# UniBwTAS/continuous_clustering

Hardware: AMD Instinct MI355X
Metric: Mpoints/s clustered (64-beam streams) (higher is better)
Workload: dtype f32

## Files before the change

### continuous_clustering_amd/__init__.py

```python
from __future__ import annotations

import ctypes as C
import os
import sys

import numpy as np

from . import capi
from .capi import Config

__all__ = ["Config", "Engine", "EngineError", "load_library", "capi", "IDENTITY_TF", "take", "TAKE_POINT_DTYPE", "TAKE_STREAM_DTYPE",
           "TakeCapacityError", "pointcloud2_fields", "TAKE_CLUSTER_DTYPE", "TAKE_CLUSTER_STREAM_DTYPE", "poses", "PoseTracks",
           "stamps", "FiringStamps", "CLUSTER_STAMP_DTYPE"]

_HERE = os.path.dirname(os.path.abspath(__file__))
LIB_PATH = os.path.join(_HERE, os.environ.get("CC_HIP_LIB", "libcc_hip.so"))
_lib = None

IDENTITY_TF = np.array([1, 0, 0, 0, 0, 1, 0, 0, 0, 0, 1, 0], dtype=np.float64)


class EngineError(RuntimeError):
    def __init__(self, code: int, msg: str):
        super().__init__(f"cc_hip error {code}: {msg}")
# ... 10 lines not shown
            return
        libdir = os.path.join(list(spec.submodule_search_locations)[0], "lib")
        for name in ("libhsa-runtime64.so", "libamdhip64.so"):
            path = os.path.join(libdir, name)
            if os.path.exists(path):
                C.CDLL(path, mode=C.RTLD_GLOBAL)
    except OSError:
        pass


def load_library():
    global _lib
    if _lib is not None:
        return _lib
    if not os.path.exists(LIB_PATH):
        raise ImportError(f"{LIB_PATH} is missing: build it with `python -m continuous_clustering_amd.build` "
                          f"(hipcc --offload-arch=gfx950); there is no CPU fallback")
    _preload_hip_runtime()
    L = C.CDLL(LIB_PATH)
    vp, i32, i64 = C.c_void_p, C.c_int, C.c_int64
    L.cc_config_default.argtypes = [C.POINTER(Config)]
    L.cc_config_default.restype = None
    L.cc_config_kitti.argtypes = [C.POINTER(Config)]
    L.cc_config_kitti.restype = None
    L.cc_version.restype = C.c_char_p
    L.cc_engine_create.argtypes = [C.POINTER(vp), i32, i32, i32, C.POINTER(Config)]
    L.cc_engine_destroy.argtypes = [vp]
    L.cc_engine_destroy.restype = None
    L.cc_engine_set_config.argtypes = [vp, C.POINTER(Config)]
    L.cc_engine_reset.argtypes = [vp, i32]
    L.cc_engine_reset_streams.argtypes = [vp, i32, vp]
    L.cc_engine_set_robot_from_sensor.argtypes = [vp, i32, vp]
    L.cc_engine_add_firings.argtypes = [vp, i32, i64, vp, vp, vp]
    L.cc_engine_add_firings_device.argtypes = [vp, i64, vp, vp, vp]
    L.cc_engine_sync.argtypes = [vp]
    L.cc_engine_inputs_released.argtypes = [vp, C.POINTER(C.c_uint64), C.POINTER(C.c_uint64)]
    L.cc_engine_hip_stream.argtypes = [vp]
    L.cc_engine_hip_stream.restype = vp
    L.cc_engine_record_events.argtypes = [vp, i32]
    L.cc_engine_drain_events.argtypes = [vp, i32, vp, i64, C.POINTER(i64)]
    L.cc_engine_pending_events.argtypes = [vp, i32, C.POINTER(i64)]
    L.cc_engine_drain_links.argtypes = [vp, i32, vp, i64, C.POINTER(i64)]
    L.cc_engine_stream_state.argtypes = [vp, i32, C.POINTER(capi.StreamState)]
    L.cc_engine_read_columns.argtypes = [vp, i32, i64, i64, C.POINTER(capi.ColumnView)]
    L.cc_engine_read_column_ranges.argtypes = [vp, i32, i32, vp, vp, C.POINTER(capi.ColumnView)]
    L.cc_engine_output_planes.argtypes = [vp, i32, C.POINTER(vp), C.POINTER(vp)]
    L.cc_engine_set_option.argtypes = [vp, C.c_char_p, i64]
    L.cc_engine_gather_cluster_points.argtypes = [vp, i32, i64, vp, vp, vp, vp, vp, vp]
    L.cc_engine_enable_timing.argtypes = [vp, i32]
    L.cc_engine_kernel_times.argtypes = [vp, C.POINTER(C.c_double * 7), C.POINTER(C.c_uint64)]
    L.cc_engine_totals.argtypes = [vp] + [C.POINTER(C.c_uint64)] * 4
    L.cc_engine_batch_counters.argtypes = [vp] + [C.POINTER(C.c_uint64)] * 2 + [C.POINTER(C.c_uint64 * 8)]
    L.cc_engine_gate_counters.argtypes = [vp] + [C.POINTER(C.c_uint64)] * 2
    L.cc_engine_resident_counters.argtypes = [vp, C.POINTER(C.c_uint64), C.POINTER(C.c_uint64), C.POINTER(C.c_int)]
    L.cc_engine_view_counters.argtypes = [vp, C.POINTER(C.c_uint64), C.POINTER(C.c_uint64)]
    L.cc_engine_last_error.argtypes = [vp]
    L.cc_engine_last_error.restype = C.c_char_p
    _lib = L
    return L


def _ptr(a):
    if a is None:
        return None
    if isinstance(a, int):
        return a
    if isinstance(a, np.ndarray):
        return a.ctypes.data
    return a.data_ptr()


class Engine:

    def __init__(self, cfg: Config, num_rows: int, num_streams: int = 1, device: int = 0, robot_from_sensor=IDENTITY_TF):
        self.L = load_library()
        self.cfg = cfg.copy()
        self.num_rows = num_rows
        self.num_streams = num_streams
        self.h = C.c_void_p()
        rc = self.L.cc_engine_create(C.byref(self.h), device, num_streams, num_rows, C.byref(self.cfg))
        if rc != capi.CC_OK:
            self.h = None
            raise EngineError(rc, "cc_engine_create failed" + (" (no MI355X visible)" if rc == capi.CC_ERR_NO_DEVICE else ""))
        if robot_from_sensor is not None:
            self.set_robot_from_sensor(robot_from_sensor)

    def close(self):
        if getattr(self, "h", None):
            self.L.cc_engine_destroy(self.h)
            self.h = None

    def __del__(self):
        try:
            self.close()
        except Exception:
            pass

    def _check(self, rc: int):
        if rc != capi.CC_OK:
            raise EngineError(rc, self.L.cc_engine_last_error(self.h).decode())

    def set_config(self, cfg: Config):
        self.cfg = cfg.copy()
        self._check(self.L.cc_engine_set_config(self.h, C.byref(self.cfg)))

    def reset(self, num_rows: int | None = None):
# ... 80 lines not shown
        a = np.ascontiguousarray(ev["a"], dtype=np.int64)
        b = np.ascontiguousarray(ev["b"], dtype=np.int64)
        cnt = np.ascontiguousarray(ev["d"], dtype=np.uint32)
        offsets = np.zeros(n + 1, dtype=np.int64)
        offsets[1:] = np.cumsum(cnt.astype(np.int64))
        gcol = np.zeros(max(1, int(offsets[-1])), dtype=np.int64)
        row = np.zeros(max(1, int(offsets[-1])), dtype=np.int32)
        self._check(self.L.cc_engine_gather_cluster_points(self.h, stream, n, cid.ctypes.data, a.ctypes.data, b.ctypes.data,
                                                           cnt.ctypes.data, gcol.ctypes.data, row.ctypes.data))
        return offsets, gcol[: offsets[-1]], row[: offsets[-1]]

    def set_option(self, name: str, value: int):
        self._check(self.L.cc_engine_set_option(self.h, name.encode(), int(value)))

    def enable_timing(self, enable: bool = True):
        self._check(self.L.cc_engine_enable_timing(self.h, 1 if enable else 0))

    def kernel_times(self) -> dict:
        ms = (C.c_double * 7)()
        n = C.c_uint64(0)
        self._check(self.L.cc_engine_kernel_times(self.h, C.byref(ms), C.byref(n)))
        names = ("prep_ms", "insert_ms", "segment_ms", "scan_ms", "assoc_lds_ms", "assoc_global_ms", "publish_ms")
        d = {k: ms[i] for i, k in enumerate(names)}
        d["batches"] = n.value
        return d

    def totals(self) -> dict:
        v = [C.c_uint64(0) for _ in range(4)]
        self._check(self.L.cc_engine_totals(self.h, *[C.byref(x) for x in v]))
        return {"cells_published": v[0].value, "clusters_finished": v[1].value, "firings_consumed": v[2].value,
                "serial_columns": v[3].value}

    def batch_counters(self) -> dict:
        v = [C.c_uint64(0) for _ in range(2)]
        why = (C.c_uint64 * 8)()
        self._check(self.L.cc_engine_batch_counters(self.h, *[C.byref(x) for x in v], C.byref(why)))
        return {"batch_columns": v[0].value, "batch_bails": v[1].value, "bail_reasons": list(why)}

    def resident_counters(self) -> dict:
        a, b, r = C.c_uint64(0), C.c_uint64(0), C.c_int(0)
        self._check(self.L.cc_engine_resident_counters(self.h, C.byref(a), C.byref(b), C.byref(r)))
        return {"launches": int(a.value), "calls": int(b.value), "running": bool(r.value)}

    def view_counters(self) -> dict:
        a, b = C.c_uint64(0), C.c_uint64(0)
        self._check(self.L.cc_engine_view_counters(self.h, C.byref(a), C.byref(b)))
        return {"mirror": int(a.value), "kernel": int(b.value)}

    def gate_counters(self) -> dict:
        v = [C.c_uint64(0) for _ in range(2)]
        self._check(self.L.cc_engine_gate_counters(self.h, *[C.byref(x) for x in v]))
        return {"lazy_batches": v[0].value, "lazy_redone": v[1].value}

    def output_planes(self, stream: int = 0):
        g, i = C.c_void_p(), C.c_void_p()
        self._check(self.L.cc_engine_output_planes(self.h, stream, C.byref(g), C.byref(i)))
        return g.value, i.value


from . import take
from .take import TAKE_POINT_DTYPE, TAKE_STREAM_DTYPE, TakeCapacityError, pointcloud2_fields
from .take import TAKE_CLUSTER_DTYPE, TAKE_CLUSTER_STREAM_DTYPE

Engine.take_points = take.take_points
Engine.take_size = take.take_size
Engine.take_cursor = take.take_cursor
Engine.take_seek = take.take_seek
Engine.take_clusters = take.take_clusters
Engine.take_clusters_size = take.take_clusters_size
Engine.take_clusters_cursor = take.take_clusters_cursor

from . import poses
from .poses import PoseTracks

from . import stamps
from .stamps import CLUSTER_STAMP_DTYPE, FiringStamps
```

### continuous_clustering_amd/csrc/cc_engine.hip

```cpp
#include <hip/hip_runtime.h>

#include <algorithm>
#include <chrono>
#include <cstdlib>
#include <cmath>
#include <cstdio>
#include <cstring>
#include <functional>
#include <limits>
#include <mutex>
#include <string>
#include <vector>

#include "cc_kernels.h"

#ifndef CC_LWAVE_MAX_STREAMS
#define CC_LWAVE_MAX_STREAMS 256
#endif

using namespace ccd;

struct cc_engine
{
    int device{0};
// ... 2651 lines not shown
    if (!e || stream < 0 || stream >= e->g.num_streams || slots < 1 || !d_original_index || !d_is_ground || !d_detection || max_points < 1 ||
        from < 0 || to - from >= e->g.ring_cols)
        return CC_ERR_INVALID_ARGUMENT;
    if (to < from)
        return CC_OK;
    (void) hipSetDevice(e->device);
    int rc = stop_resident(e);
    if (rc)
        return rc;
    rc = finish_batch(e);
    if (rc)
        return rc;
    hipLaunchKernelGGL(cck::k_scatter_apply, dim3((unsigned) (to - from + 1)), dim3(64), 0, e->stream, e->g, e->P, (const StreamState*) e->d_states, stream, (long long) from,
                       d_original_index, slots, d_is_ground, d_detection, (long long) max_points);
    CC_HIP_CHECK(e, hipGetLastError());
    return CC_OK;
}

int cc_engine_view_counters(cc_engine* e, uint64_t* served_from_mirror, uint64_t* served_by_kernel)
{
    if (!e)
        return CC_ERR_INVALID_ARGUMENT;
    if (served_from_mirror)
        *served_from_mirror = e->view_hits;
    if (served_by_kernel)
        *served_by_kernel = e->view_misses;
    return CC_OK;
}

int cc_engine_resident_counters(cc_engine* e, uint64_t* launches, uint64_t* calls, int* running)
{
    if (!e)
        return CC_ERR_INVALID_ARGUMENT;
    if (launches)
        *launches = e->res_launches;
    if (calls)
        *calls = e->res_calls + (e->res_running ? __atomic_load_n(&e->h_res_ctl->calls, __ATOMIC_ACQUIRE) : 0ull);
    if (running)
        *running = (e->res_running && __atomic_load_n(&e->h_res_ctl->exited, __ATOMIC_ACQUIRE) == 0ull) ? 1 : 0;
    return CC_OK;
}

int cc_engine_gate_counters(cc_engine* e, uint64_t* lazy_batches, uint64_t* lazy_redone)
{
    if (!e)
        return CC_ERR_INVALID_ARGUMENT;
    if (lazy_batches)
        *lazy_batches = e->lazy_batches;
    if (lazy_redone)
        *lazy_redone = e->lazy_redone;
    return CC_OK;
}

int cc_engine_batch_counters(cc_engine* e, uint64_t* batch_columns, uint64_t* batch_bails, uint64_t bail_reasons[8])
{
    if (!e)
        return CC_ERR_INVALID_ARGUMENT;
    (void) hipSetDevice(e->device);
    int rc = finish_batch(e);
    if (rc)
        return rc;
    std::vector<StreamState> st(e->g.num_streams);
    CC_HIP_CHECK(e, hipMemcpy(st.data(), e->d_states, st.size() * sizeof(StreamState), hipMemcpyDeviceToHost));
    uint64_t a = 0, b = 0;
    if (bail_reasons)
        for (int i = 0; i < 8; i++)
            bail_reasons[i] = 0;
    for (auto& s : st)
    {
        a += s.batch_columns;
        b += s.batch_bails;
        if (bail_reasons)
            for (int i = 0; i < 8; i++)
                bail_reasons[i] += s.batch_bail_reason[i];
    }
    if (bail_reasons)
        bail_reasons[7] = e->small_tail_launches;
    if (batch_columns)
        *batch_columns = a;
    if (batch_bails)
        *batch_bails = b;
    return CC_OK;
}

int cc_engine_debug_counters(cc_engine* e, int stream, uint64_t out[16])
{
    if (!e || stream < 0 || stream >= e->g.num_streams || !out)
        return CC_ERR_INVALID_ARGUMENT;
    StreamState st;
    CC_HIP_CHECK(e, hipMemcpy(&st, e->d_states + stream, sizeof(st), hipMemcpyDeviceToHost));
    for (int i = 0; i < 16; i++)
        out[i] = st.dbg[i];
    return CC_OK;
}

const char* cc_engine_last_error(cc_engine* e)
{
    return e ? e->error.c_str() : "null engine";
}

}

#include "cc_replay_eval.h"
```

### continuous_clustering_amd/csrc/cc_k_scan.h

```cpp
#pragma once

#ifndef CC_SCAN_BLOCKS
#define CC_SCAN_BLOCKS 256
#endif
constexpr int SCAN_BLOCKS = CC_SCAN_BLOCKS;

template<int RPL, bool MIRROR>
__device__ __forceinline__ void scan_body(const Geometry& g, const cc_config& cfg, const Planes& P, StreamState* states, int first_stream, int slot,
                                          const int bx, const int by, const int ny)
{
    const int s = first_stream + bx;
    const int lane = lane_id();
    const StreamState* st = &states[s];
    if (st->error != 0 || st->batch[slot].seg_begin < 0 || st->batch[slot].mode != 0)
        return;
    AssocCtx c;
    c.p = stream_ptrs(P, g, s);
    const SP& p = c.p;
    const int R = c.R = g.num_rows;
    c.NC = g.num_columns;
    const int RC = c.RC = g.ring_cols;
    c.az_width = g.az_width;
    c.maxd2 = g.max_distance_squared;
    c.max_steps_in_row = cfg.max_steps_in_row;
// ... 399 lines not shown
            visits++;
            reach = sb;
        }
        if (ccm::absf(o.w - me.w) > mad)
            next_direction(c);
        else
        {
            const float dx = me.x - o.x, dy = me.y - o.y, dz = me.z - o.z;
            if (!oign && dx * dx + dy * dy + dz * dz < c.maxd2)
            {
                const int cand = (sb << 8) | orow;
                if (!rooted)
                    parent = cand;
                else if (nlinks < LINK_SLOTS)
                {
                    packed |= (unsigned long long) cand << (16 * nlinks);
                    nlinks++;
                }
                else
                    overflow = 1;
                rooted = 1;
            }
            if (rooted && c.stop_enabled && d >= c.stop_min)
                next_direction(c);
            else
            {
                d++;
                orow = down ? orow + 1 : orow - 1;
                if (!(orow >= 0 && orow < c.R && d <= c.max_col_steps))
                    next_direction(c);
            }
        }
    }
};

constexpr int SL_CAP = 8192;
struct ScanLongRec
{
    int ci;
    int oc;
    short orow, sb, d, needed;
    short parent;
    unsigned char down, rooted, nlinks, flags;
    float mad;
    unsigned long long packed;
};
static_assert(sizeof(ScanLongRec) == 40, "long-scan record");

#ifndef CC_SCAN_CAP
#define CC_SCAN_CAP 6
#endif
constexpr int SCAN_CAP = CC_SCAN_CAP;

template<int RPL, bool MIRROR, bool SPLIT = false>
__global__ __launch_bounds__(64) void k_scan2(Geometry g, cc_config cfg, Planes P, StreamState* states, int first_stream, int slot)
{
    static_assert(!(SPLIT && MIRROR), "the long-scan list does not carry the mirror's visit counts");
    const int s = first_stream + blockIdx.x;
    const int lane = lane_id();
    const StreamState* st = &states[s];
    if (st->error != 0 || st->batch[slot].seg_begin < 0 || st->batch[slot].mode != 0)
        return;
    const SP p = stream_ptrs(P, g, s);
    const int R = g.num_rows, RC = g.ring_cols;
    ScanCfg sc;
    sc.R = R, sc.RC = RC;
    sc.maxd2 = g.max_distance_squared;
    sc.max_col_steps = cfg.max_steps_in_column;
    sc.stop_enabled = cfg.stop_after_association_enabled != 0;
    sc.stop_min = cfg.stop_after_association_min_steps;
    const int max_row_steps = cfg.max_steps_in_row;
    const int TC = SCAN_TILE_CELLS / (RPL * 64);
    __shared__ unsigned short s_list[SCAN_TILE_CELLS];
    __shared__ short s_parent[SCAN_TILE_CELLS];
    __shared__ unsigned char s_nlinks[SCAN_TILE_CELLS];
    __shared__ unsigned short s_visits[MIRROR ? SCAN_TILE_CELLS : 1];
    __shared__ unsigned char s_reach[MIRROR ? SCAN_TILE_CELLS : 1];
    __shared__ double s_fin[SCAN_TILE_CELLS];
    __shared__ unsigned long long s_links[SCAN_TILE_CELLS];
    int* const sl_ctl = P.sl_ctl + (size_t) s * 4;
    ScanLongRec* const sl_rec = (ScanLongRec*) P.sl_rec + (size_t) s * SL_CAP;
    const long long col_begin = st->batch[slot].acp_next, col_end = st->batch[slot].seg_end, first_column = st->first_column;
    const int first_lc = (int) (first_column % RC);
    const long long n_tiles = (col_end - col_begin + TC - 1) / TC;
    for (long long tile = blockIdx.y; tile < n_tiles; tile += gridDim.y)
    {
        const long long gc0 = col_begin + tile * TC;
        const int ncols = (int) (col_end - gc0 < TC ? col_end - gc0 : TC);
        const int lc0 = (int) (gc0 % RC);
        const long long rot0 = gc0 / g.num_columns;
        const int cir0 = (int) (gc0 - rot0 * g.num_columns);
        int n_act = 0;
        for (int j = 0; j < TC * RPL; j++)
        {
            const int tc = j / RPL, row = (j % RPL) * 64 + lane;
            const int tl = tc * RPL * 64 + row;
            bool act = false;
            if (tc < ncols && row < R)
            {
                int lc = lc0 + tc;
                lc = lc >= RC ? lc - RC : lc;
                act = p.ignored[lc * R + row] == 0;
            }
            s_parent[tl] = -2;
            s_nlinks[tl] = 0;
            s_fin[tl] = 0.;
            s_links[tl] = 0;
            if (MIRROR)
            {
                s_visits[tl] = 0;
                s_reach[tl] = 0;
            }
            const unsigned long long m = __ballot(act);
            if (act)
                s_list[n_act + __popcll(m & lanes_below())] = (unsigned short) tl;
            n_act += __popcll(m);
        }
        wave_lds_fence();
        unsigned deferred = 0;
        for (int base = 0; base < n_act; base += 64)
        {
            const bool have = base + lane < n_act;
            const int tl = have ? (int) s_list[base + lane] : 0;
            const int tc = tl / (RPL * 64), row = tl % (RPL * 64);
            const long long gc = gc0 + tc;
            int lc = lc0 + tc;
            lc = lc >= RC ? lc - RC : lc;
            const int ci = lc * R + row;
            ScanPoint q;
            q.me = make_float4(0.f, 0.f, 0.f, 0.f);
            q.mad = 0.f;
            q.row = row;
            double fin = 0.;
            q.needed = -1;
            if (have)
            {
                q.me = p.sc_rec[ci];
                q.mad = ccm::asinf_exact(cfg.max_distance / p.dist[ci]);
                fin = cell_caz(caz_base_of_rotation(rot0 + (cir0 + tc >= g.num_columns ? 1 : 0)), p.incaz[ci]) + (double) q.mad;
                q.needed = f2i_x86(__builtin_ceilf(q.mad / g.az_width));
                q.needed = q.needed < max_row_steps ? q.needed : max_row_steps;
            }
            q.bound = (gc - first_column) <= (long long) max_row_steps + 1 ? first_lc : -1;
            q.start(sc, have, lc);
            bool pending = false;
            if (SPLIT)
            {
                for (int it = 0; it < g.scan_cap && __any(q.run); it++)
                    if (q.run)
                        q.template step<false>(sc, p);
                const unsigned long long m = __ballot(q.run);
                if (m)
                {
                    int lbase = 0;
                    if (lane == (int) __ffsll((long long) m) - 1)
                        lbase = atomicAdd(&sl_ctl[0], (int) __popcll(m));
                    lbase = __shfl(lbase, (int) __ffsll((long long) m) - 1);
                    const int idx = lbase + (int) __popcll(m & lanes_below());
                    if (q.run && idx < g.sl_cap)
                    {
                        ScanLongRec r;
                        r.ci = ci, r.oc = q.oc;
                        r.orow = (short) q.orow, r.sb = (short) q.sb, r.d = (short) q.d, r.needed = (short) q.needed;
                        r.parent = (short) q.parent;
                        r.down = (unsigned char) q.down, r.rooted = (unsigned char) q.rooted, r.nlinks = (unsigned char) q.nlinks;
                        r.flags = (unsigned char) ((q.overflow ? 1 : 0) | (q.bound >= 0 ? 2 : 0));
                        r.mad = q.mad;
                        r.packed = q.packed;
                        sl_rec[idx] = r;
                        pending = true;
                        q.run = false;
                    }
                    while (__any(q.run))
                        if (q.run)
                            q.template step<false>(sc, p);
                }
                for (int t2 = 0; t2 < TC; t2++)
                    if (__any(pending && tc == t2))
                        deferred |= 1u << t2;
            }
            else
            {
                while (__any(q.run))
                    if (q.run)
                        q.template step<MIRROR>(sc, p);
            }
            if (have)
            {
                s_parent[tl] = (short) (pending ? -3 : q.parent);
                s_nlinks[tl] = (unsigned char) (q.overflow ? 255 : q.nlinks);
                s_fin[tl] = fin;
                s_links[tl] = q.packed;
                if (MIRROR)
                {
                    s_visits[tl] = sat_u16(q.visits);
                    s_reach[tl] = (unsigned char) q.reach;
                }
            }
        }
        wave_lds_fence();
        for (int tc = 0; tc < ncols; tc++)
        {
            int lc = lc0 + tc;
            lc = lc >= RC ? lc - RC : lc;
            int parent[RPL], nlinks[RPL];
            double fin[RPL];
            unsigned long long packed[RPL];
            int reach = 0;
            const bool later = SPLIT && ((deferred >> tc) & 1u) != 0;
#pragma unroll
            for (int k = 0; k < RPL; k++)
            {
                const int row = k * 64 + lane;
                const int tl = tc * RPL * 64 + row;
                parent[k] = s_parent[tl];
                nlinks[k] = s_nlinks[tl];
                fin[k] = s_fin[tl];
                packed[k] = s_links[tl];
                if (MIRROR)
                    reach = (int) s_reach[tl] > reach ? (int) s_reach[tl] : reach;
                if (row < R)
                {
                    const int ci = lc * R + row;
                    if (g.scan_stores_fin)
                        p.sc_fin[ci] = fin[k];
                    if (!(later && parent[k] == -3))
                    {
                        p.sc_parent[ci] = (int16_t) parent[k];
                        p.sc_nlinks[ci] = (uint8_t) nlinks[k];
                        if (nlinks[k] > 0)
                            p.sc_links[ci] = packed[k];
                    }
                    if (MIRROR)
                        p.sc_visits[ci] = s_visits[tl];
                }
            }
            if (later)
            {
                if (lane == 0)
                    p.sl_cols[atomicAdd(&sl_ctl[2], 1)] = lc;
            }
            else
                scan_column_epilogue<RPL, MIRROR>(p, R, lc, lane, parent, nlinks, fin, packed, reach);
        }
        wave_lds_fence();
    }
}

#ifndef CC_SCAN_LONG_BLOCKS
#define CC_SCAN_LONG_BLOCKS 16
#endif
constexpr int SCAN_LONG_BLOCKS = CC_SCAN_LONG_BLOCKS;
constexpr int SCAN_EPI_BLOCKS = 16;

template<int RPL>
__global__ __launch_bounds__(64) void k_scan2_long(Geometry g, cc_config cfg, Planes P, StreamState* states, int first_stream, int slot, int* __restrict__ stat)
{
    const int s = first_stream + blockIdx.x;
    int* const sl_ctl = P.sl_ctl + (size_t) s * 4;
    int n = sl_ctl[0];
    if (n <= 0)
        return;
    n = n < g.sl_cap ? n : g.sl_cap;
    const StreamState* st = &states[s];
    const int lane = lane_id();
    const SP p = stream_ptrs(P, g, s);
    const ScanLongRec* const sl_rec = (ScanLongRec*) P.sl_rec + (size_t) s * SL_CAP;
    const int R = g.num_rows, RC = g.ring_cols;
    ScanCfg sc;
    sc.R = R, sc.RC = RC;
    sc.maxd2 = g.max_distance_squared;
    sc.max_col_steps = cfg.max_steps_in_column;
    sc.stop_enabled = cfg.stop_after_association_enabled != 0;
    sc.stop_min = cfg.stop_after_association_min_steps;
    const int first_lc = (int) (st->first_column % RC);
    ScanPoint q;
    q.run = false;
    q.me = make_float4(0.f, 0.f, 0.f, 0.f);
    q.mad = 0.f, q.row = 0, q.needed = 0, q.bound = -1, q.sb = 0, q.down = 0, q.d = 0, q.oc = 0, q.orow = 0;
    q.rooted = 0, q.parent = -1, q.nlinks = 0, q.overflow = 0, q.visits = 0, q.reach = 0, q.packed = 0ull;
    int ci = 0;
    int nvis = 0;
    bool more = true;
    for (;;)
    {
        const unsigned long long idle = __ballot(!q.run);
        if (more && idle)
        {
            int lbase = 0;
            if (lane == (int) __ffsll((long long) idle) - 1)
                lbase = atomicAdd(&sl_ctl[1], (int) __popcll(idle));
            lbase = __shfl(lbase, (int) __ffsll((long long) idle) - 1);
            const int idx = lbase + (int) __popcll(idle & lanes_below());
            if (!q.run && idx < n)
            {
                const ScanLongRec r = sl_rec[idx];
                ci = r.ci;
                q.me = p.sc_rec[ci];
                q.mad = r.mad;
                q.row = ci % R;
                q.needed = r.needed;
                q.bound = (r.flags & 2) ? first_lc : -1;
                q.sb = r.sb, q.down = r.down, q.d = r.d, q.oc = r.oc, q.orow = r.orow;
                q.rooted = r.rooted, q.parent = r.parent, q.nlinks = r.nlinks, q.overflow = r.flags & 1;
                q.packed = r.packed;
                q.run = true;
            }
            more = lbase + (int) __popcll(idle) < n;
        }
        if (!__any(q.run))
            break;
        for (int it = 0; it < 8; it++)
            if (q.run)
            {
                q.template step<false>(sc, p);
                nvis++;
                if (!q.run)
                {
                    p.sc_parent[ci] = (int16_t) q.parent;
                    p.sc_nlinks[ci] = (uint8_t) (q.overflow ? 255 : q.nlinks);
                    if (q.nlinks > 0)
                        p.sc_links[ci] = q.packed;
                }
            }
    }
    if (stat)
    {
        for (int off = 32; off > 0; off >>= 1)
            nvis += __shfl_down(nvis, off, 64);
        if (lane == 0 && nvis > 0)
            atomicAdd(&stat[1], nvis);
    }
}

template<int RPL>
__global__ __launch_bounds__(64) void k_scan2_epi(Geometry g, cc_config cfg, Planes P, StreamState* states, int first_stream, int slot, int* __restrict__ stat)
{
    const int s = first_stream + blockIdx.x;
    int* const sl_ctl = P.sl_ctl + (size_t) s * 4;
    const int nd = sl_ctl[2];
    const int lane = lane_id();
    if (stat && blockIdx.y == 0 && lane == 0)
    {
        const StreamState* st = &states[s];
        if (st->error == 0 && st->batch[slot].seg_begin >= 0 && st->batch[slot].mode == 0)
        {
            atomicAdd(&stat[2], (int) (st->batch[slot].seg_end - st->batch[slot].acp_next));
        }
    }
    if (nd <= 0 && sl_ctl[0] <= 0)
        return;
    const SP p = stream_ptrs(P, g, s);
    const int R = g.num_rows;
    for (int i = blockIdx.y; i < nd; i += gridDim.y)
    {
        const int lc = p.sl_cols[i];
        const CazBase cb = caz_base_of_column(p.colg[lc], g.num_columns);
        int parent[RPL], nlinks[RPL];
        double fin[RPL];
        unsigned long long packed[RPL];
#pragma unroll
        for (int k = 0; k < RPL; k++)
        {
            const int row = k * 64 + lane;
            parent[k] = -2, nlinks[k] = 0, fin[k] = 0., packed[k] = 0ull;
            if (row < R)
            {
                const int ci = lc * R + row;
                parent[k] = p.sc_parent[ci];
                nlinks[k] = p.sc_nlinks[ci];
                fin[k] = cell_fin(cfg, p, ci, cb);
                if (nlinks[k] > 0)
                    packed[k] = p.sc_links[ci];
            }
        }
        scan_column_epilogue<RPL, false>(p, R, lc, lane, parent, nlinks, fin, packed, 0);
    }
    __threadfence();
    if (lane == 0 && atomicAdd(&sl_ctl[3], 1) == (int) gridDim.y - 1)
    {
        sl_ctl[0] = 0;
        sl_ctl[1] = 0;
        sl_ctl[2] = 0;
        sl_ctl[3] = 0;
    }
}
```

### continuous_clustering_amd/csrc/cc_launch.h

```cpp
#define CC_TARGS(...) __VA_ARGS__
#define CC_LAUNCH_RPL_T(kern_, targs_, rpl_, grid_, block_, lds_, st_, ...)               \
    do                                                                                     \
    {                                                                                      \
        if ((rpl_) == 1)                                                                   \
            hipLaunchKernelGGL((kern_<1 targs_>), grid_, block_, lds_, st_, __VA_ARGS__); \
        else                                                                               \
            hipLaunchKernelGGL((kern_<2 targs_>), grid_, block_, lds_, st_, __VA_ARGS__); \
    } while (0)
#define CC_LAUNCH_RPL(kern_, rpl_, ...) CC_LAUNCH_RPL_T(kern_, , rpl_, __VA_ARGS__)
#define CC_LAUNCH_RPL_MIRROR(kern_, rpl_, mirror_, ...)                   \
    do                                                                    \
    {                                                                     \
        if (mirror_)                                                      \
            CC_LAUNCH_RPL_T(kern_, CC_TARGS(, true), rpl_, __VA_ARGS__);  \
        else                                                              \
            CC_LAUNCH_RPL_T(kern_, CC_TARGS(, false), rpl_, __VA_ARGS__); \
    } while (0)

struct BatchPass
{
    hipStream_t si, sb, sc, sa, sp;
    int slot, first_stream, count;
    int64_t n;
    const float* d_xyz;
// ... 190 lines not shown
    bool lwave;
    int scan_stores_fin;
};

static AssocPlan plan_association(cc_engine* e, const BatchPass& bp, const bool small_front)
{
    const int count = bp.count;
    bool batch_assoc = e->assoc_batch && e->cfg.cluster_point_trees_every_nth_column == 1;
    if (batch_assoc && e->assoc_rounds == 0 && e->h_bail_count && !e->capturing && count >= 8)
    {
        const int seen_now = *e->h_bail_count;
        if (e->chronic_skip > 0)
        {
            e->chronic_skip--;
            e->bail_seen = seen_now;
            batch_assoc = false;
            if (e->chronic_skip == 0)
                e->bail_cooldown = e->bail_cooldown_batches > 2 ? e->bail_cooldown_batches : 2;
        }
        else if ((seen_now - e->chronic_seen) * 4 >= count && e->chronic_probe)
            e->chronic_skip = 8;
        e->chronic_probe = batch_assoc;
        e->chronic_seen = seen_now;
    }
    int adaptive_rounds = 1;
    if (e->assoc_rounds == 0 && e->h_bail_count && !e->capturing)
    {
        const int seen = *e->h_bail_count;
        if (seen != e->bail_seen)
        {
            e->bail_seen = seen;
            e->bail_cooldown = e->bail_cooldown_batches;
        }
        if (e->bail_cooldown > 0)
        {
            e->bail_cooldown--;
            adaptive_rounds = 3;
        }
    }
    AssocPlan plan{batch_assoc, batch_assoc ? (e->assoc_rounds > 0 ? e->assoc_rounds : adaptive_rounds) : 1, count, false, 0};
    const bool idle_net = batch_assoc && e->assoc_rounds == 0 && adaptive_rounds == 1;
    if (idle_net && !e->capturing && e->assoc_sweep_blocks < count)
        plan.blocks = e->assoc_sweep_blocks;
    plan.lwave = e->assoc_waves == 4 || (e->assoc_waves_auto && count <= CC_LWAVE_MAX_STREAMS);
    plan.scan_stores_fin = (!small_front && !idle_net) ? 1 : 0;
    if (e->scan_store_fin >= 0 && !small_front)
        plan.scan_stores_fin = e->scan_store_fin;
    return plan;
}

struct ScanChoice
{
    bool packed, split;
};

static ScanChoice choose_scan(cc_engine* e, const BatchPass& bp)
{
    const int rpl = bp.rpl, count = bp.count;
    const bool packed_default = e->scan_packed == 1 || (e->scan_packed < 0 && (rpl > 1 || count > 192));
    if (e->g.mirror_fields || e->scan_split == 0)
        return {packed_default, false};
    if (e->scan_split == 1 || !e->h_bail_count || e->capturing)
        return {packed_default, packed_default && e->scan_split == 1};
    const unsigned vis = (unsigned) e->h_bail_count[1], cols = (unsigned) e->h_bail_count[2];
    const unsigned dc = cols - e->split_cols_seen, dv = vis - e->split_rec_seen;
    if (dc >= 1024u)
    {
        const double rate = (double) dv / ((double) dc * (double) rpl);
        e->split_on = e->split_on ? rate > 20.0 : rate > 40.0;
        e->split_cols_seen = cols, e->split_rec_seen = vis;
    }
    const bool probe = (e->split_probe++ & 31u) == 0u;
    const bool promote = !packed_default && e->scan_packed < 0 && rpl == 1 && count >= 48;
    const bool split = (e->split_on || probe) && (packed_default || promote);
    return {packed_default || (promote && split), split};
}

static int launch_scan(cc_engine* e, const BatchPass& bp, const ScanChoice scan, const Geometry& gs)
{
    const Geometry& g = e->g;
    const hipStream_t sc = bp.sc;
    const dim3 scan_grid((unsigned) bp.count, cck::SCAN_BLOCKS);
    if (scan.packed && scan.split)
    {
        const dim3 long_grid((unsigned) bp.count, cck::SCAN_LONG_BLOCKS), epi_grid((unsigned) bp.count, cck::SCAN_EPI_BLOCKS);
        CC_LAUNCH_RPL_T(cck::k_scan2, CC_TARGS(, false, true), bp.rpl, scan_grid, dim3(64), 0, sc, gs, e->cfg, e->P, e->d_states, bp.first_stream, bp.slot);
        CC_LAUNCH_RPL(cck::k_scan2_long, bp.rpl, long_grid, dim3(64), 0, sc, g, e->cfg, e->P, e->d_states, bp.first_stream, bp.slot, e->d_bail_count);
        CC_LAUNCH_RPL(cck::k_scan2_epi, bp.rpl, epi_grid, dim3(64), 0, sc, g, e->cfg, e->P, e->d_states, bp.first_stream, bp.slot, e->d_bail_count);
    }
    else if (scan.packed)
        CC_LAUNCH_RPL_MIRROR(cck::k_scan2, bp.rpl, g.mirror_fields, scan_grid, dim3(64), 0, sc, gs, e->cfg, e->P, e->d_states, bp.first_stream, bp.slot);
    else
        CC_LAUNCH_RPL_MIRROR(cck::k_scan, bp.rpl, g.mirror_fields, scan_grid, dim3(64), 0, sc, gs, e->cfg, e->P, e->d_states, bp.first_stream, bp.slot);
    CC_MARK(EV_SCAN, sc);
    if (sc != bp.sa)
    {
        CC_HIP_CHECK(e, hipEventRecord(e->ev_seg[bp.slot], sc));
        CC_HIP_CHECK(e, hipStreamWaitEvent(bp.sa, e->ev_seg[bp.slot], 0));
    }
    return CC_OK;
}

static void launch_assocb(cc_engine* e, const BatchPass& bp)
{
    CC_LAUNCH_RPL(cck::k_assocb, bp.rpl, dim3(bp.count), dim3(cck::AB_THREADS), 0, bp.sa, e->g, e->cfg, e->P, e->d_states, bp.first_stream, bp.slot,
                  e->d_bail_count);
}

static int launch_association(cc_engine* e, const BatchPass& bp, const AssocPlan& plan, const Geometry& gs)
{
    const hipStream_t sa = bp.sa;
    const int count = bp.count;
    CC_MARK(EV_CHAIN3, sa);
    bool marked7 = false;
    bool global_done = false;
    if (e->assoc_waves >= 2 && e->cfg.cluster_point_trees_every_nth_column == 1)
    {
        const dim3 block(plan.lwave ? cck::A3_THREADS : 192);
        for (int r = 0; r < plan.rounds; r++)
        {
            if (plan.batch_assoc)
            {
                launch_assocb(e, bp);
                if (r == 0)
                {
                    CC_MARK(EV_ASSOC_LDS, sa);
                    marked7 = true;
                }
            }
            const int limited = r + 1 < plan.rounds ? 1 : 0;
            CC_LAUNCH_RPL(cck::k_assoc3, bp.rpl, dim3(plan.blocks), block, 0, sa, gs, e->cfg, e->P, e->d_states, bp.first_stream, bp.slot, limited, count, 1);
            global_done = limited == 0;
        }
    }
    else
    {
        if (plan.batch_assoc)
        {
            launch_assocb(e, bp);
            CC_MARK(EV_ASSOC_LDS, sa);
            marked7 = true;
        }
        CC_LAUNCH_RPL(cck::k_assoc_lds, bp.rpl, dim3(count), dim3(64), 0, sa, gs, e->cfg, e->P, e->d_states, bp.first_stream, bp.slot);
    }
// ... 230 lines not shown
```

### include/cc_hip.h

```cpp
#ifndef CC_HIP_H
#define CC_HIP_H

#include <stdint.h>

#ifdef __cplusplus
extern "C" {
#endif

enum
{
    CC_OK = 0,
    CC_ERR_INVALID_ARGUMENT = 1,
    CC_ERR_HIP = 2,
    CC_ERR_NO_DEVICE = 3,
    CC_ERR_FIRING_SIZE = 4,
    CC_ERR_NO_ROBOT_TRANSFORM = 5,
    CC_ERR_RING_OVERRUN = 6,
    CC_ERR_BOOKKEEPING = 7,
    CC_ERR_CAPACITY = 8,
    CC_ERR_NEGATIVE_COLUMN = 9
};

enum
{
// ... 169 lines not shown
    uint8_t  intensity;
    uint32_t column;
} cc_take_point;

typedef struct cc_take_stream {
    int64_t col_from, col_to;
    int64_t lost_columns;
    int64_t first_record, n_records;
    int32_t error;
    int32_t pad;
} cc_take_stream;

int cc_engine_take_points(cc_engine* e, int stage, int select, cc_take_point* d_records, int64_t capacity,
                          cc_take_stream* d_table , cc_take_stream* h_table ,
                          int64_t* n_records);
int cc_engine_take_cursor(cc_engine* e, int stage, int stream, int64_t* cursor, int64_t* readable_from);
int cc_engine_take_seek(cc_engine* e, int stage, int stream , int64_t column);

typedef struct cc_take_cluster {
    int32_t  stream;
    uint32_t id;
    int64_t  col_from;
    int64_t  first_record;
    uint32_t n_points, n_columns;
    uint32_t firing_min, firing_max;
    float    min_x, min_y, min_z, max_x, max_y, max_z;
} cc_take_cluster;

typedef struct cc_take_cluster_stream {
    int64_t id_from, id_to;
    int64_t lost_columns;
    int64_t first_record, n_records;
    int32_t first_cluster, n_clusters;
    int32_t error;
    int32_t pad;
} cc_take_cluster_stream;

enum { CC_TAKE_CLUSTERS_WITH_POINTS = 0, CC_TAKE_CLUSTERS_DESCRIPTORS_ONLY = 1 };

int cc_engine_take_clusters(cc_engine* e, uint32_t min_points, int flags,
                            cc_take_cluster* d_clusters, int64_t cluster_capacity,
                            cc_take_point* d_records, int64_t record_capacity,
                            cc_take_cluster_stream* d_table , cc_take_cluster_stream* h_table ,
                            int64_t* n_clusters, int64_t* n_records);
int cc_engine_take_clusters_cursor(cc_engine* e, int stream, int64_t* next_id, int64_t* floor_column, int64_t* readable_from);

int cc_engine_set_option(cc_engine* e, const char* name, int64_t value);

int cc_engine_enable_timing(cc_engine* e, int enable);
int cc_engine_kernel_times(cc_engine* e, double ms[7], uint64_t* launches);
int cc_engine_totals(cc_engine* e, uint64_t* cells_published, uint64_t* clusters_finished, uint64_t* firings_consumed,
                     uint64_t* serial_columns);
int cc_engine_batch_counters(cc_engine* e, uint64_t* batch_columns, uint64_t* batch_bails, uint64_t bail_reasons[8]);
int cc_engine_resident_counters(cc_engine* e, uint64_t* launches, uint64_t* calls, int* running);
int cc_engine_view_counters(cc_engine* e, uint64_t* served_from_mirror, uint64_t* served_by_kernel);

int cc_engine_gate_counters(cc_engine* e, uint64_t* lazy_batches, uint64_t* lazy_redone);

typedef struct cc_eval_frame_result
{
    double tp, fn, fp, tn;
    double over_segmentation_entropy;
    double under_segmentation_entropy;
} cc_eval_frame_result;

int cc_eval_frame(int device, int64_t n, const uint16_t* semantic, const uint32_t* euclid, const uint8_t* is_ground,
                  const uint32_t* detection, cc_eval_frame_result* out);
int cc_eval_frame_device(int64_t n, const uint16_t* d_semantic, const uint32_t* d_euclid, const uint8_t* d_is_ground,
                         const uint32_t* d_detection, cc_eval_frame_result* out);
void cc_eval_mean_std(const double* data, int64_t n, double* mean, double* std_dev);
void cc_eval_summarize(const cc_eval_frame_result* frames, int64_t n, double out[12]);

int cc_eval_gather_records(void* nccl_comm, int world, int device, const double* records, int64_t n, int64_t capacity, double* out,
                           int64_t* counts);

int cc_eval_generate_euclidean_labels(int device, int64_t n, const float* points, const uint16_t* semantic, const uint16_t* instance,
                                      uint16_t* out_labels);

const char* cc_engine_last_error(cc_engine* e);
const char* cc_version(void);

#ifdef __cplusplus
}
#endif
#endif
```

Baseline: 19860.

## Add pooled multi-wave scan kernel that drains long scans in shared memory

```diff
diff --git a/continuous_clustering_amd/__init__.py b/continuous_clustering_amd/__init__.py
--- a/continuous_clustering_amd/__init__.py
+++ b/continuous_clustering_amd/__init__.py
@@ -86,6 +86,8 @@
     L.cc_engine_totals.argtypes = [vp] + [C.POINTER(C.c_uint64)] * 4
     L.cc_engine_batch_counters.argtypes = [vp] + [C.POINTER(C.c_uint64)] * 2 + [C.POINTER(C.c_uint64 * 8)]
     L.cc_engine_gate_counters.argtypes = [vp] + [C.POINTER(C.c_uint64)] * 2
+    if hasattr(L, "cc_engine_scan_counters"):
+        L.cc_engine_scan_counters.argtypes = [vp] + [C.POINTER(C.c_uint64)] * 2
     L.cc_engine_resident_counters.argtypes = [vp, C.POINTER(C.c_uint64), C.POINTER(C.c_uint64), C.POINTER(C.c_int)]
     L.cc_engine_view_counters.argtypes = [vp, C.POINTER(C.c_uint64), C.POINTER(C.c_uint64)]
     L.cc_engine_last_error.argtypes = [vp]
@@ -272,6 +274,11 @@
         self._check(self.L.cc_engine_gate_counters(self.h, *[C.byref(x) for x in v]))
         return {"lazy_batches": v[0].value, "lazy_redone": v[1].value}
 
+    def scan_counters(self) -> dict:
+        v = [C.c_uint64(0) for _ in range(2)]
+        self._check(self.L.cc_engine_scan_counters(self.h, *[C.byref(x) for x in v]))
+        return {"long_scan_visits": v[0].value, "columns": v[1].value}
+
     def output_planes(self, stream: int = 0):
         g, i = C.c_void_p(), C.c_void_p()
         self._check(self.L.cc_engine_output_planes(self.h, stream, C.byref(g), C.byref(i)))
diff --git a/continuous_clustering_amd/csrc/cc_engine.hip b/continuous_clustering_amd/csrc/cc_engine.hip
--- a/continuous_clustering_amd/csrc/cc_engine.hip
+++ b/continuous_clustering_amd/csrc/cc_engine.hip
@@ -2727,6 +2727,23 @@
     return CC_OK;
 }
 
+int cc_engine_scan_counters(cc_engine* e, uint64_t* long_scan_visits, uint64_t* columns)
+{
+    if (!e)
+        return CC_ERR_INVALID_ARGUMENT;
+    (void) hipSetDevice(e->device);
+    int rc = finish_batch(e);
+    if (rc)
+        return rc;
+    int c[4] = {0, 0, 0, 0};
+    CC_HIP_CHECK(e, hipMemcpy(c, e->d_bail_count, sizeof(c), hipMemcpyDeviceToHost));
+    if (long_scan_visits)
+        *long_scan_visits = (uint64_t) (uint32_t) c[1];
+    if (columns)
+        *columns = (uint64_t) (uint32_t) c[2];
+    return CC_OK;
+}
+
 int cc_engine_batch_counters(cc_engine* e, uint64_t* batch_columns, uint64_t* batch_bails, uint64_t bail_reasons[8])
 {
     if (!e)
diff --git a/continuous_clustering_amd/csrc/cc_k_scan.h b/continuous_clustering_amd/csrc/cc_k_scan.h
--- a/continuous_clustering_amd/csrc/cc_k_scan.h
+++ b/continuous_clustering_amd/csrc/cc_k_scan.h
@@ -475,38 +475,203 @@
 #endif
 constexpr int SCAN_CAP = CC_SCAN_CAP;
 
-template<int RPL, bool MIRROR, bool SPLIT = false>
-__global__ __launch_bounds__(64) void k_scan2(Geometry g, cc_config cfg, Planes P, StreamState* states, int first_stream, int slot)
-{
-    static_assert(!(SPLIT && MIRROR), "the long-scan list does not carry the mirror's visit counts");
-    const int s = first_stream + blockIdx.x;
-    const int lane = lane_id();
-    const StreamState* st = &states[s];
-    if (st->error != 0 || st->batch[slot].seg_begin < 0 || st->batch[slot].mode != 0)
-        return;
-    const SP p = stream_ptrs(P, g, s);
-    const int R = g.num_rows, RC = g.ring_cols;
+#ifndef CC_SCAN_POOL
+#define CC_SCAN_POOL 1
+#endif
+#ifndef CC_SCAN_POOL_WAVES
+#define CC_SCAN_POOL_WAVES 4
+#endif
+#ifndef CC_SCAN_POOL_RECORDS
+#define CC_SCAN_POOL_RECORDS 128
+#endif
+constexpr int SCAN_POOL_WAVES = CC_SCAN_POOL_WAVES;
+constexpr int SCAN_POOL_RECORDS = CC_SCAN_POOL_RECORDS;
+#ifndef CC_SCAN_POOL_BLOCKS
+#define CC_SCAN_POOL_BLOCKS 8
+#endif
+constexpr int SCAN_POOL_BLOCKS = CC_SCAN_POOL_BLOCKS;
+static_assert((SCAN_POOL_WAVES & (SCAN_POOL_WAVES - 1)) == 0 && SCAN_POOL_WAVES >= 1 && SCAN_POOL_WAVES <= 16 && SCAN_POOL_BLOCKS >= 1, "pooled block");
+enum
+{
+    PL_NREC = 0,
+    PL_NEXT = 1,
+    PL_NCOLS = 2,
+    PL_NVIS = 3,
+    PL_TILE = 4,
+    PL_GO = 5,
+    PL_WORDS = 8
+};
+
+__device__ __forceinline__ ScanCfg scan_cfg_of(const Geometry& g, const cc_config& cfg)
+{
     ScanCfg sc;
-    sc.R = R, sc.RC = RC;
+    sc.R = g.num_rows, sc.RC = g.ring_cols;
     sc.maxd2 = g.max_distance_squared;
     sc.max_col_steps = cfg.max_steps_in_column;
     sc.stop_enabled = cfg.stop_after_association_enabled != 0;
     sc.stop_min = cfg.stop_after_association_min_steps;
+    return sc;
+}
+
+__device__ __forceinline__ ScanLongRec scan_long_record(const ScanPoint& q, const int ci)
+{
+    ScanLongRec r;
+    r.ci = ci, r.oc = q.oc;
+    r.orow = (short) q.orow, r.sb = (short) q.sb, r.d = (short) q.d, r.needed = (short) q.needed;
+    r.parent = (short) q.parent;
+    r.down = (unsigned char) q.down, r.rooted = (unsigned char) q.rooted, r.nlinks = (unsigned char) q.nlinks;
+    r.flags = (unsigned char) ((q.overflow ? 1 : 0) | (q.bound >= 0 ? 2 : 0));
+    r.mad = q.mad;
+    r.packed = q.packed;
+    return r;
+}
+
+__device__ __forceinline__ int scan_long_drain(const ScanCfg& sc, const SP& p, const ScanLongRec* const rec, const int n, int* const next, const int first_lc,
+                                               const int lane)
+{
+    const int R = sc.R;
+    ScanPoint q;
+    q.run = false;
+    q.me = make_float4(0.f, 0.f, 0.f, 0.f);
+    q.mad = 0.f, q.row = 0, q.needed = 0, q.bound = -1, q.sb = 0, q.down = 0, q.d = 0, q.oc = 0, q.orow = 0;
+    q.rooted = 0, q.parent = -1, q.nlinks = 0, q.overflow = 0, q.visits = 0, q.reach = 0, q.packed = 0ull;
+    int ci = 0;
+    int nvis = 0;
+    bool more = n > 0;
+    for (;;)
+    {
+        const unsigned long long idle = __ballot(!q.run);
+        if (more && idle)
+        {
+            int lbase = 0;
+            if (lane == (int) __ffsll((long long) idle) - 1)
+                lbase = atomicAdd(next, (int) __popcll(idle));
+            lbase = __shfl(lbase, (int) __ffsll((long long) idle) - 1);
+            const int idx = lbase + (int) __popcll(idle & lanes_below());
+            if (!q.run && idx < n)
+            {
+                const ScanLongRec r = rec[idx];
+                ci = r.ci;
+                q.me = p.sc_rec[ci];
+                q.mad = r.mad;
+                q.row = ci % R;
+                q.needed = r.needed;
+                q.bound = (r.flags & 2) ? first_lc : -1;
+                q.sb = r.sb, q.down = r.down, q.d = r.d, q.oc = r.oc, q.orow = r.orow;
+                q.rooted = r.rooted, q.parent = r.parent, q.nlinks = r.nlinks, q.overflow = r.flags & 1;
+                q.packed = r.packed;
+                q.run = true;
+            }
+            more = lbase + (int) __popcll(idle) < n;
+        }
+        if (!__any(q.run))
+            break;
+        for (int it = 0; it < 8; it++)
+            if (q.run)
+            {
+                q.template step<false>(sc, p);
+                nvis++;
+                if (!q.run)
+                {
+                    p.sc_parent[ci] = (int16_t) q.parent;
+                    p.sc_nlinks[ci] = (uint8_t) (q.overflow ? 255 : q.nlinks);
+                    if (q.nlinks > 0)
+                        p.sc_links[ci] = q.packed;
+                }
+            }
+    }
+    return nvis;
+}
+
+template<int RPL>
+__device__ __forceinline__ void scan_deferred_epilogue(const Geometry& g, const cc_config& cfg, const SP& p, const int lc, const int lane)
+{
+    const int R = g.num_rows;
+    const CazBase cb = caz_base_of_column(p.colg[lc], g.num_columns);
+    int parent[RPL], nlinks[RPL];
+    double fin[RPL];
+    unsigned long long packed[RPL];
+#pragma unroll
+    for (int k = 0; k < RPL; k++)
+    {
+        const int row = k * 64 + lane;
+        parent[k] = -2, nlinks[k] = 0, fin[k] = 0., packed[k] = 0ull;
+        if (row < R)
+        {
+            const int ci = lc * R + row;
+            parent[k] = p.sc_parent[ci];
+            nlinks[k] = p.sc_nlinks[ci];
+            fin[k] = cell_fin(cfg, p, ci, cb);
+            if (nlinks[k] > 0)
+                packed[k] = p.sc_links[ci];
+        }
+    }
+    scan_column_epilogue<RPL, false>(p, R, lc, lane, parent, nlinks, fin, packed, 0);
+}
+
+template<int RPL, bool MIRROR, bool SPLIT = false, bool POOL = false>
+__global__ __launch_bounds__(POOL ? 64 * SCAN_POOL_WAVES : 64) void k_scan2(Geometry g, cc_config cfg, Planes P, StreamState* states, int first_stream, int slot,
+                                                                           int* __restrict__ stat)
+{
+    static_assert(!(SPLIT && MIRROR), "the long-scan list does not carry the mirror's visit counts");
+    static_assert(!(POOL && (MIRROR || SPLIT)), "the pooled form is the packed form without the mirror's fields, in place of the three-kernel split");
+    constexpr int WV = POOL ? SCAN_POOL_WAVES : 1;
+    const int s = first_stream + blockIdx.x;
+    const int lane = lane_id();
+    const int wave = POOL ? uniform_i32((int) (threadIdx.x >> 6)) : 0;
+    const StreamState* st = &states[s];
+    __shared__ unsigned short s_list_w[WV][SCAN_TILE_CELLS];
+    __shared__ short s_parent_w[WV][SCAN_TILE_CELLS];
+    __shared__ unsigned char s_nlinks_w[WV][SCAN_TILE_CELLS];
+    __shared__ unsigned short s_visits_w[WV][MIRROR ? SCAN_TILE_CELLS : 1];
+    __shared__ unsigned char s_reach_w[WV][MIRROR ? SCAN_TILE_CELLS : 1];
+    __shared__ double s_fin_w[WV][SCAN_TILE_CELLS];
+    __shared__ unsigned long long s_links_w[WV][SCAN_TILE_CELLS];
+    __shared__ ScanLongRec s_rec[POOL ? SCAN_POOL_RECORDS : 1];
+    __shared__ int s_cols[POOL ? SCAN_POOL_RECORDS : 1];
+    __shared__ int s_ctl[POOL ? PL_WORDS : 1];
+    if constexpr (POOL)
+    {
+        if (threadIdx.x == 0)
+        {
+            s_ctl[PL_NREC] = 0, s_ctl[PL_NEXT] = 0, s_ctl[PL_NCOLS] = 0, s_ctl[PL_NVIS] = 0, s_ctl[PL_TILE] = 0;
+            s_ctl[PL_GO] = (st->error != 0 || st->batch[slot].seg_begin < 0 || st->batch[slot].mode != 0) ? 0 : 1;
+        }
+        __syncthreads();
+        if (s_ctl[PL_GO] == 0)
+            return;
+    }
+    else
+    {
+        if (st->error != 0 || st->batch[slot].seg_begin < 0 || st->batch[slot].mode != 0)
+            return;
+    }
+    unsigned short* const s_list = s_list_w[wave];
+    short* const s_parent = s_parent_w[wave];
+    unsigned char* const s_nlinks = s_nlinks_w[wave];
+    unsigned short* const s_visits = s_visits_w[wave];
+    unsigned char* const s_reach = s_reach_w[wave];
+    double* const s_fin = s_fin_w[wave];
+    unsigned long long* const s_links = s_links_w[wave];
+    const SP p = stream_ptrs(P, g, s);
+    const int R = g.num_rows, RC = g.ring_cols;
+    const ScanCfg sc = scan_cfg_of(g, cfg);
     const int max_row_steps = cfg.max_steps_in_row;
     const int TC = SCAN_TILE_CELLS / (RPL * 64);
-    __shared__ unsigned short s_list[SCAN_TILE_CELLS];
-    __shared__ short s_parent[SCAN_TILE_CELLS];
-    __shared__ unsigned char s_nlinks[SCAN_TILE_CELLS];
-    __shared__ unsigned short s_visits[MIRROR ? SCAN_TILE_CELLS : 1];
-    __shared__ unsigned char s_reach[MIRROR ? SCAN_TILE_CELLS : 1];
-    __shared__ double s_fin[SCAN_TILE_CELLS];
-    __shared__ unsigned long long s_links[SCAN_TILE_CELLS];
     int* const sl_ctl = P.sl_ctl + (size_t) s * 4;
     ScanLongRec* const sl_rec = (ScanLongRec*) P.sl_rec + (size_t) s * SL_CAP;
+    const int list_cap = POOL ? (g.sl_cap < SCAN_POOL_RECORDS ? g.sl_cap : SCAN_POOL_RECORDS) : g.sl_cap;
     const long long col_begin = st->batch[slot].acp_next, col_end = st->batch[slot].seg_end, first_column = st->first_column;
     const int first_lc = (int) (first_column % RC);
     const long long n_tiles = (col_end - col_begin + TC - 1) / TC;
-    for (long long tile = blockIdx.y; tile < n_tiles; tile += gridDim.y)
+    auto pool_tile = [&]() -> long long {
+        int k = 0;
+        if (lane == 0)
+            k = atomicAdd(&s_ctl[PL_TILE], 1);
+        k = uniform_i32(k);
+        return (long long) (k / WV) * ((long long) gridDim.y * WV) + (long long) blockIdx.y * WV + (k % WV);
+    };
+    for (long long tile = POOL ? pool_tile() : (long long) blockIdx.y; tile < n_tiles; tile = POOL ? pool_tile() : tile + gridDim.y)
     {
         const long long gc0 = col_begin + tile * TC;
         const int ncols = (int) (col_end - gc0 < TC ? col_end - gc0 : TC);
@@ -567,7 +732,7 @@
             q.bound = (gc - first_column) <= (long long) max_row_steps + 1 ? first_lc : -1;
             q.start(sc, have, lc);
             bool pending = false;
-            if (SPLIT)
+            if (SPLIT || POOL)
             {
                 for (int it = 0; it < g.scan_cap && __any(q.run); it++)
                     if (q.run)
@@ -577,20 +742,15 @@
                 {
                     int lbase = 0;
                     if (lane == (int) __ffsll((long long) m) - 1)
-                        lbase = atomicAdd(&sl_ctl[0], (int) __popcll(m));
+                        lbase = POOL ? atomicAdd(&s_ctl[PL_NREC], (int) __popcll(m)) : atomicAdd(&sl_ctl[0], (int) __popcll(m));
                     lbase = __shfl(lbase, (int) __ffsll((long long) m) - 1);
                     const int idx = lbase + (int) __popcll(m & lanes_below());
-                    if (q.run && idx < g.sl_cap)
+                    if (q.run && idx < list_cap)
                     {
-                        ScanLongRec r;
-                        r.ci = ci, r.oc = q.oc;
-                        r.orow = (short) q.orow, r.sb = (short) q.sb, r.d = (short) q.d, r.needed = (short) q.needed;
-                        r.parent = (short) q.parent;
-                        r.down = (unsigned char) q.down, r.rooted = (unsigned char) q.rooted, r.nlinks = (unsigned char) q.nlinks;
-                        r.flags = (unsigned char) ((q.overflow ? 1 : 0) | (q.bound >= 0 ? 2 : 0));
-                        r.mad = q.mad;
-                        r.packed = q.packed;
-                        sl_rec[idx] = r;
+                        if (POOL)
+                            s_rec[idx] = scan_long_record(q, ci);
+                        else
+                            sl_rec[idx] = scan_long_record(q, ci);
                         pending = true;
                         q.run = false;
                     }
@@ -630,7 +790,7 @@
             double fin[RPL];
             unsigned long long packed[RPL];
             int reach = 0;
-            const bool later = SPLIT && ((deferred >> tc) & 1u) != 0;
+            const bool later = (SPLIT || POOL) && ((deferred >> tc) & 1u) != 0;
 #pragma unroll
             for (int k = 0; k < RPL; k++)
             {
@@ -661,12 +821,38 @@
             if (later)
             {
                 if (lane == 0)
-                    p.sl_cols[atomicAdd(&sl_ctl[2], 1)] = lc;
+                {
+                    if (POOL)
+                        s_cols[atomicAdd(&s_ctl[PL_NCOLS], 1)] = lc;
+                    else
+                        p.sl_cols[atomicAdd(&sl_ctl[2], 1)] = lc;
+                }
             }
             else
                 scan_column_epilogue<RPL, MIRROR>(p, R, lc, lane, parent, nlinks, fin, packed, reach);
         }
         wave_lds_fence();
+    }
+    if constexpr (POOL)
+    {
+        __syncthreads();
+        const int asked = s_ctl[PL_NREC];
+        int nvis = scan_long_drain(sc, p, s_rec, asked < list_cap ? asked : list_cap, &s_ctl[PL_NEXT], first_lc, lane);
+        for (int off = 32; off > 0; off >>= 1)
+            nvis += __shfl_down(nvis, off, 64);
+        if (lane == 0 && nvis > 0)
+            atomicAdd(&s_ctl[PL_NVIS], nvis);
+        __syncthreads();
+        const int nd = s_ctl[PL_NCOLS];
+        for (int i = wave; i < nd; i += WV)
+            scan_deferred_epilogue<RPL>(g, cfg, p, s_cols[i], lane);
+        if (stat && threadIdx.x == 0)
+        {
+            if (s_ctl[PL_NVIS] > 0)
+                atomicAdd(&stat[1], s_ctl[PL_NVIS]);
+            if (blockIdx.y == 0)
+                atomicAdd(&stat[2], (int) (col_end - col_begin));
+        }
     }
 }
 
@@ -689,64 +875,8 @@
     const int lane = lane_id();
     const SP p = stream_ptrs(P, g, s);
     const ScanLongRec* const sl_rec = (ScanLongRec*) P.sl_rec + (size_t) s * SL_CAP;
-    const int R = g.num_rows, RC = g.ring_cols;
-    ScanCfg sc;
-    sc.R = R, sc.RC = RC;
-    sc.maxd2 = g.max_distance_squared;
-    sc.max_col_steps = cfg.max_steps_in_column;
-    sc.stop_enabled = cfg.stop_after_association_enabled != 0;
-    sc.stop_min = cfg.stop_after_association_min_steps;
-    const int first_lc = (int) (st->first_column % RC);
-    ScanPoint q;
-    q.run = false;
-    q.me = make_float4(0.f, 0.f, 0.f, 0.f);
-    q.mad = 0.f, q.row = 0, q.needed = 0, q.bound = -1, q.sb = 0, q.down = 0, q.d = 0, q.oc = 0, q.orow = 0;
-    q.rooted = 0, q.parent = -1, q.nlinks = 0, q.overflow = 0, q.visits = 0, q.reach = 0, q.packed = 0ull;
-    int ci = 0;
-    int nvis = 0;
-    bool more = true;
-    for (;;)
-    {
-        const unsigned long long idle = __ballot(!q.run);
-        if (more && idle)
-        {
-            int lbase = 0;
-            if (lane == (int) __ffsll((long long) idle) - 1)
-                lbase = atomicAdd(&sl_ctl[1], (int) __popcll(idle));
-            lbase = __shfl(lbase, (int) __ffsll((long long) idle) - 1);
-            const int idx = lbase + (int) __popcll(idle & lanes_below());
-            if (!q.run && idx < n)
-            {
-                const ScanLongRec r = sl_rec[idx];
-                ci = r.ci;
-                q.me = p.sc_rec[ci];
-                q.mad = r.mad;
-                q.row = ci % R;
-                q.needed = r.needed;
-                q.bound = (r.flags & 2) ? first_lc : -1;
-                q.sb = r.sb, q.down = r.down, q.d = r.d, q.oc = r.oc, q.orow = r.orow;
-                q.rooted = r.rooted, q.parent = r.parent, q.nlinks = r.nlinks, q.overflow = r.flags & 1;
-                q.packed = r.packed;
-                q.run = true;
-            }
-            more = lbase + (int) __popcll(idle) < n;
-        }
-        if (!__any(q.run))
-            break;
-        for (int it = 0; it < 8; it++)
-            if (q.run)
-            {
-                q.template step<false>(sc, p);
-                nvis++;
-                if (!q.run)
-                {
-                    p.sc_parent[ci] = (int16_t) q.parent;
-                    p.sc_nlinks[ci] = (uint8_t) (q.overflow ? 255 : q.nlinks);
-                    if (q.nlinks > 0)
-                        p.sc_links[ci] = q.packed;
-                }
-            }
-    }
+    const ScanCfg sc = scan_cfg_of(g, cfg);
+    int nvis = scan_long_drain(sc, p, sl_rec, n, &sl_ctl[1], (int) (st->first_column % g.ring_cols), lane);
     if (stat)
     {
         for (int off = 32; off > 0; off >>= 1)
@@ -774,31 +904,8 @@
     if (nd <= 0 && sl_ctl[0] <= 0)
         return;
     const SP p = stream_ptrs(P, g, s);
-    const int R = g.num_rows;
     for (int i = blockIdx.y; i < nd; i += gridDim.y)
-    {
-        const int lc = p.sl_cols[i];
-        const CazBase cb = caz_base_of_column(p.colg[lc], g.num_columns);
-        int parent[RPL], nlinks[RPL];
-        double fin[RPL];
-        unsigned long long packed[RPL];
-#pragma unroll
-        for (int k = 0; k < RPL; k++)
-        {
-            const int row = k * 64 + lane;
-            parent[k] = -2, nlinks[k] = 0, fin[k] = 0., packed[k] = 0ull;
-            if (row < R)
-            {
-                const int ci = lc * R + row;
-                parent[k] = p.sc_parent[ci];
-                nlinks[k] = p.sc_nlinks[ci];
-                fin[k] = cell_fin(cfg, p, ci, cb);
-                if (nlinks[k] > 0)
-                    packed[k] = p.sc_links[ci];
-            }
-        }
-        scan_column_epilogue<RPL, false>(p, R, lc, lane, parent, nlinks, fin, packed, 0);
-    }
+        scan_deferred_epilogue<RPL>(g, cfg, p, p.sl_cols[i], lane);
     __threadfence();
     if (lane == 0 && atomicAdd(&sl_ctl[3], 1) == (int) gridDim.y - 1)
     {
diff --git a/continuous_clustering_amd/csrc/cc_launch.h b/continuous_clustering_amd/csrc/cc_launch.h
--- a/continuous_clustering_amd/csrc/cc_launch.h
+++ b/continuous_clustering_amd/csrc/cc_launch.h
@@ -266,6 +266,7 @@
 struct ScanChoice
 {
     bool packed, split;
+    bool pool;
 };
 
 static ScanChoice choose_scan(cc_engine* e, const BatchPass& bp)
@@ -273,9 +274,9 @@
     const int rpl = bp.rpl, count = bp.count;
     const bool packed_default = e->scan_packed == 1 || (e->scan_packed < 0 && (rpl > 1 || count > 192));
     if (e->g.mirror_fields || e->scan_split == 0)
-        return {packed_default, false};
+        return {packed_default, false, packed_default && !e->g.mirror_fields && CC_SCAN_POOL != 0};
     if (e->scan_split == 1 || !e->h_bail_count || e->capturing)
-        return {packed_default, packed_default && e->scan_split == 1};
+        return {packed_default, packed_default && e->scan_split == 1, false};
     const unsigned vis = (unsigned) e->h_bail_count[1], cols = (unsigned) e->h_bail_count[2];
     const unsigned dc = cols - e->split_cols_seen, dv = vis - e->split_rec_seen;
     if (dc >= 1024u)
@@ -287,7 +288,7 @@
     const bool probe = (e->split_probe++ & 31u) == 0u;
     const bool promote = !packed_default && e->scan_packed < 0 && rpl == 1 && count >= 48;
     const bool split = (e->split_on || probe) && (packed_default || promote);
-    return {packed_default || (promote && split), split};
+    return {packed_default || (promote && split), split, false};
 }
 
 static int launch_scan(cc_engine* e, const BatchPass& bp, const ScanChoice scan, const Geometry& gs)
@@ -298,12 +299,20 @@
     if (scan.packed && scan.split)
     {
         const dim3 long_grid((unsigned) bp.count, cck::SCAN_LONG_BLOCKS), epi_grid((unsigned) bp.count, cck::SCAN_EPI_BLOCKS);
-        CC_LAUNCH_RPL_T(cck::k_scan2, CC_TARGS(, false, true), bp.rpl, scan_grid, dim3(64), 0, sc, gs, e->cfg, e->P, e->d_states, bp.first_stream, bp.slot);
+        CC_LAUNCH_RPL_T(cck::k_scan2, CC_TARGS(, false, true), bp.rpl, scan_grid, dim3(64), 0, sc, gs, e->cfg, e->P, e->d_states, bp.first_stream, bp.slot,
+                        (int*) nullptr);
         CC_LAUNCH_RPL(cck::k_scan2_long, bp.rpl, long_grid, dim3(64), 0, sc, g, e->cfg, e->P, e->d_states, bp.first_stream, bp.slot, e->d_bail_count);
         CC_LAUNCH_RPL(cck::k_scan2_epi, bp.rpl, epi_grid, dim3(64), 0, sc, g, e->cfg, e->P, e->d_states, bp.first_stream, bp.slot, e->d_bail_count);
     }
+    else if (scan.packed && scan.pool)
+    {
+        const dim3 pool_grid((unsigned) bp.count, cck::SCAN_POOL_BLOCKS);
+        CC_LAUNCH_RPL_T(cck::k_scan2, CC_TARGS(, false, false, true), bp.rpl, pool_grid, dim3(64 * cck::SCAN_POOL_WAVES), 0, sc, gs, e->cfg, e->P, e->d_states,
+                        bp.first_stream, bp.slot, e->d_bail_count);
+    }
     else if (scan.packed)
-        CC_LAUNCH_RPL_MIRROR(cck::k_scan2, bp.rpl, g.mirror_fields, scan_grid, dim3(64), 0, sc, gs, e->cfg, e->P, e->d_states, bp.first_stream, bp.slot);
+        CC_LAUNCH_RPL_MIRROR(cck::k_scan2, bp.rpl, g.mirror_fields, scan_grid, dim3(64), 0, sc, gs, e->cfg, e->P, e->d_states, bp.first_stream, bp.slot,
+                             (int*) nullptr);
     else
         CC_LAUNCH_RPL_MIRROR(cck::k_scan, bp.rpl, g.mirror_fields, scan_grid, dim3(64), 0, sc, gs, e->cfg, e->P, e->d_states, bp.first_stream, bp.slot);
     CC_MARK(EV_SCAN, sc);
diff --git a/include/cc_hip.h b/include/cc_hip.h
--- a/include/cc_hip.h
+++ b/include/cc_hip.h
@@ -245,6 +245,7 @@
 int cc_engine_totals(cc_engine* e, uint64_t* cells_published, uint64_t* clusters_finished, uint64_t* firings_consumed,
                      uint64_t* serial_columns);
 int cc_engine_batch_counters(cc_engine* e, uint64_t* batch_columns, uint64_t* batch_bails, uint64_t bail_reasons[8]);
+int cc_engine_scan_counters(cc_engine* e, uint64_t* long_scan_visits, uint64_t* columns);
 int cc_engine_resident_counters(cc_engine* e, uint64_t* launches, uint64_t* calls, int* running);
 int cc_engine_view_counters(cc_engine* e, uint64_t* served_from_mirror, uint64_t* served_by_kernel);
 
```

New measurement: 19730. About the same (-0.6%).
